# wildminder/ComfyUI-KEEP

Hardware: AMD Instinct MI355X
Metric: restored 512x512 face frames/sec, T=20 clip (higher is better)
Workload: dtype f16x3; 1 GPU; 48 independent clips x T=20 x 512x512 per GPU (BASELINE configs[1] clips), KEEP config, synthetic weights seed 0, precision policy x3; clips_per_gpu=48, clip_length=20, parallelism=dp1 over clips, precision_policy=x3

## Files before the change

comfyui-keep_amd/csrc/keep_conv_x3.hip:

```cpp
#include <stdlib.h>

#include "keep_conv_common.h"

typedef _Float16 f16x8 __attribute__((ext_vector_type(8)));
typedef _Float16 f16x4 __attribute__((ext_vector_type(4)));
typedef unsigned int u32x4 __attribute__((ext_vector_type(4)));
typedef float f32x2 __attribute__((ext_vector_type(2)));
typedef _Float16 f16x2 __attribute__((ext_vector_type(2)));

__device__ __forceinline__ void split4(const float (&v)[4], f16x4& hi, f16x4& lo) {
#pragma unroll
  for (int j = 0; j < 4; ++j) {
    const _Float16 h = (_Float16)v[j];
    hi[j] = h;
    lo[j] = (_Float16)(v[j] - (float)h);
  }
}

template <int PRO, bool FAST>
__device__ __forceinline__ float pro_x3(float v) {
  return FAST ? pro_apply_x3(v, PRO) : pro_apply(v, PRO);
}

typedef unsigned int u32x2 __attribute__((ext_vector_type(2)));
// ... 661 lines not shown
    if (a_mv[it] && (!ONE || p.in_amax || !PLAIN)) {
      a_n[it] = (int)(m / hw);
      const int r = (int)(m - (long)a_n[it] * hw);
      a_oy[it] = r / p.Wo;
      a_ox[it] = r - a_oy[it] * p.Wo;
      if (p.in_amax) {
        float inv;
        x3_range_scale(p.in_amax[a_n[it]], a_s[it], inv);
      }
    }
  }
  const long wrow_stride = (long)p.KH * p.KW * p.Cin * (X1 ? 1 : 2);
  const int b_col = X1 ? (b_pc & 3) * 8 : ((b_pc & 3) >> 1) * XBK + (b_pc >> 2) * 16 + (b_pc & 1) * 8;

  struct StepRegs {
    float a_raw[A_IT][8];
    bool a_ok[A_IT];
    uint4 b_raw[B_IT];
    int a_c;
    float u_sc[8], u_sh[8];
  };
  const long m_last = (m0 + BM - 1 < p.M) ? (m0 + BM - 1) : (long)p.M - 1;
  const bool uni_n = !PLAIN && p.pro_scale && ((m0 / hw) == (m_last / hw));
  const long uni_off = (m0 / hw) * (long)p.Cin;

  const long rows_here = (p.M - m0) < BM ? (p.M - m0) : BM;
  __amdgpu_buffer_rsrc_t a_rsrc = __builtin_amdgcn_make_buffer_rsrc((void*)p.in, 0, 0, 0x00020000);
  int a_voff[A_IT];
  if (ONE) {
    const unsigned long long b = (unsigned long long)(p.in + m0 * p.in_ld);
    const unsigned lo = __builtin_amdgcn_readfirstlane((unsigned)b), hi = __builtin_amdgcn_readfirstlane((unsigned)(b >> 32));
    a_rsrc = __builtin_amdgcn_make_buffer_rsrc((void*)(((unsigned long long)hi << 32) | lo), 0, (int)rows_here * p.in_ld * 4, 0x00020000);
#pragma unroll
    for (int it = 0; it < A_IT; ++it) a_voff[it] = ((a_row0 + it * 64) * p.in_ld + a_grp * 8) * 4;
  }
  __amdgpu_buffer_rsrc_t a2_rsrc = a_rsrc;
  int a2_voff[A_IT];
  const int ld2 = p.Cin - p.cin1;
  if (ONE && p.in2) {
    const unsigned long long b = (unsigned long long)(p.in2 + m0 * ld2);
    const unsigned lo = __builtin_amdgcn_readfirstlane((unsigned)b), hi = __builtin_amdgcn_readfirstlane((unsigned)(b >> 32));
    a2_rsrc = __builtin_amdgcn_make_buffer_rsrc((void*)(((unsigned long long)hi << 32) | lo), 0, (int)rows_here * ld2 * 4, 0x00020000);
#pragma unroll
    for (int it = 0; it < A_IT; ++it) a2_voff[it] = ((a_row0 + it * 64) * ld2 + a_grp * 8) * 4;
  }
  const __amdgpu_buffer_rsrc_t w_rsrc =
      __builtin_amdgcn_make_buffer_rsrc((void*)p.wx3, 0, p.Cout * p.KH * p.KW * p.Cin * (X1 ? 2 : 4), 0x00020000);
  int b_voff[B_IT];
#pragma unroll
  for (int it = 0; it < B_IT; ++it) {
    const int co = n0 + b_row0 + it * 32;
    b_voff[it] = (co < p.Cout && !(X1 && b_pc >= 4)) ? (int)((long)co * wrow_stride * 2) + b_pc * 16 : (int)0x80000000;
  }

  auto fetch = [&](int s, StepRegs& R) {
    const int tap = s / cchunks;
    const int c0 = (s - tap * cchunks) * XBK;
    const int kh = tap / p.KW;
    const int kw = tap - kh * p.KW;
    const int ca = c0 + a_grp * 8;
    R.a_c = ca;
    if (uni_n && ca < p.Cin) {
#pragma unroll
      for (int j = 0; j < 8; ++j) {
        R.u_sc[j] = p.pro_scale[uni_off + ca + j];
        R.u_sh[j] = p.pro_shift[uni_off + ca + j];
      }
    }
    if (ONE) {
#pragma unroll
      for (int it = 0; it < A_IT; ++it) {
        R.a_ok[it] = ca < p.Cin;
        const bool second = p.in2 && c0 >= p.cin1;
        u32x4 v0, v1;
        if (KEEP_LD_AUX_GEMM_A1 != 0 && BN >= 128 && p.Cout <= BN && !p.in2) {
          v0 = __builtin_amdgcn_raw_buffer_load_b128(a_rsrc, a_voff[it], c0 * 4, KEEP_LD_AUX_GEMM_A1);
          v1 = __builtin_amdgcn_raw_buffer_load_b128(a_rsrc, a_voff[it] + 16, c0 * 4, KEEP_LD_AUX_GEMM_A1);
        } else {
          v0 = second ? __builtin_amdgcn_raw_buffer_load_b128(a2_rsrc, a2_voff[it], (c0 - p.cin1) * 4, 0)
                      : __builtin_amdgcn_raw_buffer_load_b128(a_rsrc, a_voff[it], c0 * 4, 0);
          v1 = second ? __builtin_amdgcn_raw_buffer_load_b128(a2_rsrc, a2_voff[it] + 16, (c0 - p.cin1) * 4, 0)
                      : __builtin_amdgcn_raw_buffer_load_b128(a_rsrc, a_voff[it] + 16, c0 * 4, 0);
        }
        R.a_raw[it][0] = __uint_as_float(v0.x); R.a_raw[it][1] = __uint_as_float(v0.y);
        R.a_raw[it][2] = __uint_as_float(v0.z); R.a_raw[it][3] = __uint_as_float(v0.w);
        R.a_raw[it][4] = __uint_as_float(v1.x); R.a_raw[it][5] = __uint_as_float(v1.y);
        R.a_raw[it][6] = __uint_as_float(v1.z); R.a_raw[it][7] = __uint_as_float(v1.w);
      }
    } else {
#pragma unroll
      for (int it = 0; it < A_IT; ++it) {
        int iy = a_oy[it] * p.stride - p.pad_t + kh;
        int ix = a_ox[it] * p.stride - p.pad_l + kw;
        KEEP_REFLECT(iy, ix, p.H, p.W)
        R.a_ok[it] = a_mv[it] && iy >= 0 && iy < p.H && ix >= 0 && ix < p.W && ca < p.Cin;
        if (R.a_ok[it]) {
          const float* src = p.in + (((long)a_n[it] * p.H + iy) * p.W + ix) * p.in_ld + ca;
          const float4 v0 = *reinterpret_cast<const float4*>(src);
          const float4 v1 = *reinterpret_cast<const float4*>(src + 4);
          R.a_raw[it][0] = v0.x; R.a_raw[it][1] = v0.y; R.a_raw[it][2] = v0.z; R.a_raw[it][3] = v0.w;
          R.a_raw[it][4] = v1.x; R.a_raw[it][5] = v1.y; R.a_raw[it][6] = v1.z; R.a_raw[it][7] = v1.w;
        }
      }
    }
    const bool cb_ok = X1 ? c0 + (b_pc & 3) * 8 < p.Cin : c0 + (b_pc >> 2) * 16 < p.Cin;
#pragma unroll
    for (int it = 0; it < B_IT; ++it) {
      const u32x4 v = __builtin_amdgcn_raw_buffer_load_b128(w_rsrc, cb_ok ? b_voff[it] : (int)0x80000000, (tap * p.Cin + c0) * (X1 ? 2 : 4), 0);
      R.b_raw[it] = make_uint4(v.x, v.y, v.z, v.w);
    }
  };

  auto stage = [&](int buf, StepRegs& R) {
#pragma unroll
    for (int it = 0; it < A_IT; ++it) {
      f16x8 hi, lo;
      if (R.a_ok[it]) {
        float v[8];
#pragma unroll
        for (int j = 0; j < 8; ++j) v[j] = R.a_raw[it][j];
        if (!PLAIN) {
          if (uni_n) {
#pragma unroll
            for (int j = 0; j < 8; ++j) v[j] = v[j] * R.u_sc[j] + R.u_sh[j];
          } else if (p.pro_scale) {
            const float* sc = p.pro_scale + (long)a_n[it] * p.Cin + R.a_c;
            const float* sh = p.pro_shift + (long)a_n[it] * p.Cin + R.a_c;
#pragma unroll
            for (int j = 0; j < 8; ++j) v[j] = v[j] * sc[j] + sh[j];
          }
          if (p.pro_act != KEEP_PRO_NONE) {
#pragma unroll
            for (int j = 0; j < 8; ++j) v[j] = p.fast ? pro_apply_x3(v[j], p.pro_act) : pro_apply(v[j], p.pro_act);
          }
        }
#pragma unroll
        for (int j = 0; j < 8; j += 2) {
          const f32x2 vs = f32x2{v[j], v[j + 1]} * a_s[it];
          const f16x2 h = __builtin_convertvector(vs, f16x2);
          hi[j] = h.x; hi[j + 1] = h.y;
          if constexpr (!X1) {
            const f16x2 l = __builtin_convertvector(vs - __builtin_convertvector(h, f32x2), f16x2);
            lo[j] = l.x; lo[j + 1] = l.y;
          }
        }
      } else {
#pragma unroll
        for (int j = 0; j < 8; ++j) { hi[j] = (_Float16)0.f; lo[j] = (_Float16)0.f; }
      }
      _Float16* dst = &As[buf][(a_row0 + it * 64) * XP + a_grp * 8];
      *reinterpret_cast<f16x8*>(dst) = hi;
      if constexpr (!X1) *reinterpret_cast<f16x8*>(dst + XBK) = lo;
    }
    if (X1 && b_pc >= 4) return;
#pragma unroll
    for (int it = 0; it < B_IT; ++it)
      *reinterpret_cast<uint4*>(&Bs[buf][(b_row0 + it * 32) * XP + b_col]) = R.b_raw[it];
  };

  f32x16 acc[TM][TN];
#pragma unroll
  for (int i = 0; i < TM; ++i)
#pragma unroll
    for (int j = 0; j < TN; ++j)
#pragma unroll
      for (int r = 0; r < 16; ++r) acc[i][j][r] = 0.f;

  const int l31 = lane & 31;
  const int lhi = lane >> 5;
  const int a_f0 = (wm * TM * 32 + l31) * XP + lhi * 8;
  const int b_f0 = (wn * TN * 32 + l31) * XP + lhi * 8;

  auto mma_step = [&](int buf, bool zc = false) {
    const _Float16* Ab = As[buf];
    const _Float16* Bb = Bs[buf];
#pragma unroll
    for (int ks = 0; ks < XBK / 16; ++ks) {
      f16x8 ah[TM], al[TM], bh[TN], bl[TN];
#pragma unroll
      for (int i = 0; i < TM; ++i) {
        ah[i] = *reinterpret_cast<const f16x8*>(Ab + a_f0 + i * 32 * XP + ks * 16);
        if constexpr (!X1) al[i] = *reinterpret_cast<const f16x8*>(Ab + a_f0 + i * 32 * XP + ks * 16 + XBK);
      }
#pragma unroll
      for (int j = 0; j < TN; ++j) {
        bh[j] = *reinterpret_cast<const f16x8*>(Bb + b_f0 + j * 32 * XP + ks * 16);
        if constexpr (!X1) bl[j] = *reinterpret_cast<const f16x8*>(Bb + b_f0 + j * 32 * XP + ks * 16 + XBK);
      }
#pragma unroll
      for (int i = 0; i < TM; ++i)
#pragma unroll
        for (int j = 0; j < TN; ++j) {
          if constexpr (X1) {
            acc[i][j] = __builtin_amdgcn_mfma_f32_32x32x16_f16(ah[i], bh[j], acc[i][j], 0, 0, 0);
          } else if (KAL && zc && ks == 0) {
            const f32x16 z16 = {0.f, 0.f, 0.f, 0.f, 0.f, 0.f, 0.f, 0.f, 0.f, 0.f, 0.f, 0.f, 0.f, 0.f, 0.f, 0.f};
            acc[i][j] = __builtin_amdgcn_mfma_f32_32x32x16_f16(al[i], bh[j], z16, 0, 0, 0);
            acc[i][j] = __builtin_amdgcn_mfma_f32_32x32x16_f16(ah[i], bl[j], acc[i][j], 0, 0, 0);
            acc[i][j] = __builtin_amdgcn_mfma_f32_32x32x16_f16(ah[i], bh[j], acc[i][j], 0, 0, 0);
          } else {
            MMA_X3(acc[i][j], ah[i], al[i], bh[j], bl[j])
          }
        }
    }
  };

  if (s_begin < s_end) {
    constexpr int PD = (TM * TN == 1 && DEEP) ? (PLAIN ? 4 : 2) : 1;
    StepRegs R[PD];
#pragma unroll
    for (int u = 0; u < PD; ++u)
      if (s_begin + u < s_end) fetch(s_begin + u, R[u]);
    stage(0, R[0]);
    __syncthreads();
    int buf = 0;
    f32x16 tot[KSL ? TM : 1][KSL ? TN : 1];
    int ksl_left = p.kslice_steps;
    bool ksl_first = true;
    for (int s0 = s_begin; s0 < s_end; s0 += PD) {
#pragma unroll
      for (int u = 0; u < PD; ++u) {
        const int s = s0 + u;
        if (s < s_end) {
          if (s + PD < s_end) fetch(s + PD, R[u]);
          if (KAL) {
            mma_step(buf, u == 0);
            if (u == PD - 1) {
              if (ksl_first) {
#pragma unroll
                for (int i = 0; i < TM; ++i)
#pragma unroll
                  for (int j = 0; j < TN; ++j) tot[KSL ? i : 0][KSL ? j : 0] = acc[i][j];
              } else {
#pragma unroll
                for (int i = 0; i < TM; ++i)
#pragma unroll
                  for (int j = 0; j < TN; ++j)
#pragma unroll
                    for (int r = 0; r < 16; ++r) tot[KSL ? i : 0][KSL ? j : 0][r] += acc[i][j][r];
              }
              ksl_first = false;
            }
          } else {
            mma_step(buf);
          }
          if (KSL && !KAL && --ksl_left == 0) {
            ksl_left = p.kslice_steps;
#pragma unroll
            for (int i = 0; i < TM; ++i)
#pragma unroll
              for (int j = 0; j < TN; ++j)
#pragma unroll
                for (int r = 0; r < 16; ++r) {
                  tot[KSL ? i : 0][KSL ? j : 0][r] = ksl_first ? acc[i][j][r] : tot[KSL ? i : 0][KSL ? j : 0][r] + acc[i][j][r];
                  acc[i][j][r] = 0.f;
                }
            ksl_first = false;
          }
          if (s + 1 < s_end) stage(buf ^ 1, R[(u + 1) % PD]);
          __syncthreads();
          buf ^= 1;
        }
      }
    }
    if (KSL) {
#pragma unroll
      for (int i = 0; i < TM; ++i)
#pragma unroll
        for (int j = 0; j < TN; ++j) acc[i][j] = tot[KSL ? i : 0][KSL ? j : 0];
    }
  }
  const float asc = p.acc_scale;
  if (p.in_amax) {
#pragma unroll
    for (int i = 0; i < TM; ++i)
#pragma unroll
      for (int r = 0; r < 16; ++r) {
        const long m = m0 + wm * TM * 32 + i * 32 + (r & 3) + 8 * (r >> 2) + 4 * lhi;
        float sr = 1.f, inv = 1.f;
        if (m < p.M) x3_range_scale(p.in_amax[m / hw], sr, inv);
#pragma unroll
        for (int j = 0; j < TN; ++j) acc[i][j][r] *= asc * inv;
      }
  } else {
#pragma unroll
    for (int i = 0; i < TM; ++i)
#pragma unroll
      for (int j = 0; j < TN; ++j)
#pragma unroll
        for (int r = 0; r < 16; ++r) acc[i][j][r] *= asc;
  }
  if (m0 + BM <= p.M && p.Cout * 4L * BM < (1L << 30) && p.out_ld * 4L * BM < (1L << 30) && p.res_ld * 4L * BM < (1L << 30)) {
    if (p.split_k == 1 && !p.aux && p.epi_act == KEEP_ACT_NONE)
      x3_gather_epilogue<WGM, WGN, TM, TN, true>(p, acc, reinterpret_cast<float*>(smem_b), m0, n0, wm, wn, lane, wave, z);
    else
      x3_gather_epilogue<WGM, WGN, TM, TN, false>(p, acc, reinterpret_cast<float*>(smem_b), m0, n0, wm, wn, lane, wave, z);
    return;
  }
  staged_epilogue<WGM, WGN, TM, TN>(p, acc, reinterpret_cast<float*>(smem_b), m0, n0, wm, wn, lane, wave, z);
}

#define C3X_K 32
#define C3X_P 72
__global__ __launch_bounds__(256, 2) void conv3x3_c3_x3_kernel(ConvP p, int tiles_x, int tiles_y, int ncb, int n_items) {
  constexpr int HW_ = 34, HROWS = 10;
  constexpr int EPI_B = 4 * 64 * 68 * 4;
  constexpr int A_B = 256 * C3X_P * 2;
  static_assert(A_B + HROWS * HW_ * 4 * 4 <= EPI_B, "im2col rows + halo fit the staging area");
  __shared__ __attribute__((aligned(16))) unsigned char lds_raw[EPI_B + 64 * C3X_P * 2];
  float* et_base = reinterpret_cast<float*>(lds_raw);
  _Float16* As = reinterpret_cast<_Float16*>(lds_raw);
  float* Hs = reinterpret_cast<float*>(lds_raw + A_B);
  _Float16* Ws = reinterpret_cast<_Float16*>(lds_raw + EPI_B);

  const int tid = threadIdx.x;
  const int lane = tid & 63;
  const int wave = tid >> 6;
  const int l31 = lane & 31, lhi = lane >> 5;
  const int Cin = p.Cin, K = 9 * Cin;
  const int rowf = HW_ * Cin;

  int cur_cb = -1;
  auto load_weights = [&](int cb) {
    for (int i = tid; i < 64 * C3X_K; i += 256) {
      const int co = i >> 5, k = i & 31;
      float v = 0.f;
      if (k < K && cb * 64 + co < p.Cout) v = p.w[(long)(cb * 64 + co) * K + k];
      const _Float16 h = (_Float16)v;
      Ws[co * C3X_P + k] = h;
      Ws[co * C3X_P + 32 + k] = (_Float16)(v - (float)h);
    }
  };

  f32x16 acc[2][2];
  const bool has_act = p.epi_act != KEEP_ACT_NONE;
  const int py = tid >> 5, px = tid & 31;
  struct Item { int cb, tx, ty, n; };
  auto decode = [&](int item) {
    Item it;
    const int lid = xcd_remap(item, n_items);
    it.cb = lid % ncb;
    int t = lid / ncb;
    it.tx = t % tiles_x; t /= tiles_x;
    it.ty = t % tiles_y;
    it.n = t / tiles_y;
    return it;
  };
  constexpr int HV = (HROWS * HW_ * 3 + 255) / 256;
  float hv[HV], amax_raw = 0.f;
  auto load_halo = [&](const Item& it) {
    const float* img = p.in + (long)it.n * p.H * p.W * p.in_ld;
    const int oy0 = it.ty * 8, ox0 = it.tx * 32;
#pragma unroll
    for (int u = 0; u < HV; ++u) {
      const int i = tid + u * 256;
      hv[u] = 0.f;
      if (i < HROWS * rowf) {
        const int hy = i / rowf, r = i - hy * rowf;
        const int hx = r / Cin, c = r - hx * Cin;
        const int iy = oy0 - 1 + hy, ix = ox0 - 1 + hx;
        if (iy >= 0 && iy < p.H && ix >= 0 && ix < p.W) hv[u] = img[((long)iy * p.W + ix) * p.in_ld + c];
      }
    }
    if (p.in_amax) amax_raw = p.in_amax[it.n];
  };
  int amax_n = -1;
  float amax_seen = 0.f;
  int item = blockIdx.x;
  if (item >= n_items) return;
  Item nxt = decode(item);
  load_halo(nxt);
  for (; item < n_items; item += gridDim.x) {
    const Item cur = nxt;
    const int cb = cur.cb, tx = cur.tx, ty = cur.ty, n = cur.n;
    const int oy0 = ty * 8, ox0 = tx * 32, n0 = cb * 64;
    float in_s = 1.f, in_inv = 1.f;
    if (p.in_amax) x3_range_scale(amax_raw, in_s, in_inv);
    __syncthreads();
    if (cb != cur_cb) {
      load_weights(cb);
      cur_cb = cb;
    }
#pragma unroll
    for (int u = 0; u < HV; ++u)
      if (tid + u * 256 < HROWS * rowf) Hs[tid + u * 256] = hv[u] * in_s;
    if (item + (int)gridDim.x < n_items) {
      nxt = decode(item + gridDim.x);
      load_halo(nxt);
    }
    __syncthreads();
    {
      float vals[C3X_K];
#pragma unroll
      for (int k = 0; k < C3X_K; ++k) vals[k] = 0.f;
#pragma unroll
      for (int kh = 0; kh < 3; ++kh)
#pragma unroll
        for (int kwc = 0; kwc < 9; ++kwc)
          if (kwc < 3 * Cin && kh * 3 * Cin + kwc < C3X_K) vals[kh * 3 * Cin + kwc] = Hs[(py + kh) * rowf + px * Cin + kwc];
      f16x8 hi[4], lo[4];
#pragma unroll
      for (int k = 0; k < C3X_K; ++k) {
        const _Float16 h = (_Float16)vals[k];
        hi[k >> 3][k & 7] = h;
        lo[k >> 3][k & 7] = (_Float16)(vals[k] - (float)h);
      }
      __syncthreads();
#pragma unroll
      for (int q = 0; q < 4; ++q) {
        *reinterpret_cast<f16x8*>(&As[tid * C3X_P + q * 8]) = hi[q];
        *reinterpret_cast<f16x8*>(&As[tid * C3X_P + 32 + q * 8]) = lo[q];
      }
    }
    __syncthreads();
#pragma unroll
    for (int i = 0; i < 2; ++i)
#pragma unroll
      for (int j = 0; j < 2; ++j)
#pragma unroll
        for (int r = 0; r < 16; ++r) acc[i][j][r] = 0.f;
#pragma unroll
    for (int ks = 0; ks < 2; ++ks) {
      f16x8 ah[2], al[2], bh[2], bl[2];
#pragma unroll
      for (int i = 0; i < 2; ++i) {
        const _Float16* src = &As[(wave * 64 + i * 32 + l31) * C3X_P + ks * 16 + lhi * 8];
        ah[i] = *reinterpret_cast<const f16x8*>(src);
        al[i] = *reinterpret_cast<const f16x8*>(src + 32);
      }
#pragma unroll
      for (int j = 0; j < 2; ++j) {
        const _Float16* src = &Ws[(j * 32 + l31) * C3X_P + ks * 16 + lhi * 8];
        bh[j] = *reinterpret_cast<const f16x8*>(src);
        bl[j] = *reinterpret_cast<const f16x8*>(src + 32);
      }
#pragma unroll
      for (int i = 0; i < 2; ++i)
#pragma unroll
        for (int j = 0; j < 2; ++j) {
          MMA_X3(acc[i][j], ah[i], al[i], bh[j], bl[j])
        }
    }
    __syncthreads();
    constexpr int EP = 68;
    float* et = et_base + wave * 64 * EP;
#pragma unroll
    for (int i = 0; i < 2; ++i)
#pragma unroll
      for (int j = 0; j < 2; ++j)
#pragma unroll
        for (int r = 0; r < 16; ++r) et[(i * 32 + (r & 3) + 8 * (r >> 2) + 4 * lhi) * EP + j * 32 + l31] = acc[i][j][r] * in_inv;
    __builtin_amdgcn_s_waitcnt(0xc07f);
    const int c4 = (lane & 15) * 4, prow = lane >> 4;
    const int co = n0 + c4;
    const bool cok = co < p.Cout;
    float s4[4] = {0.f, 0.f, 0.f, 0.f}, ss4[4] = {0.f, 0.f, 0.f, 0.f};
    float amx = 0.f;
    float4 bias4 = make_float4(0.f, 0.f, 0.f, 0.f);
    if (p.bias && cok) bias4 = *reinterpret_cast<const float4*>(p.bias + co);
#pragma unroll 8
    for (int q16 = 0; q16 < 16; ++q16) {
      if (!cok) break;
      const int pxl = q16 * 4 + prow;
      const int oy = oy0 + 2 * wave + (pxl >> 5);
      const long m = ((long)n * p.Ho + oy) * p.Wo + ox0 + (pxl & 31);
      const float4 v = *reinterpret_cast<const float4*>(et + pxl * EP + c4);
      float e[4] = {v.x + bias4.x, v.y + bias4.y, v.z + bias4.z, v.w + bias4.w};
      if (has_act) {
#pragma unroll
        for (int q = 0; q < 4; ++q) e[q] = p.fast ? act_apply_fast(e[q], p.epi_act) : act_apply(e[q], p.epi_act);
      }
      if (KEEP_NT_C3)
        __builtin_nontemporal_store((f32x4){e[0], e[1], e[2], e[3]}, reinterpret_cast<f32x4*>(p.out + m * p.out_ld + co));
      else
        *reinterpret_cast<float4*>(p.out + m * p.out_ld + co) = make_float4(e[0], e[1], e[2], e[3]);
#pragma unroll
      for (int q = 0; q < 4; ++q) {
        s4[q] += e[q];
        ss4[q] += e[q] * e[q];
        amx = fmaxf(amx, fabsf(e[q]));
      }
    }
    if (p.out_amax) {
      if (n != amax_n) {
        amax_n = n;
        amax_seen = 0.f;
      }
      if (__builtin_amdgcn_ballot_w64(amx > amax_seen) != 0ull) {
        unsigned b = __float_as_uint(amx);
#pragma unroll
        for (int o = 32; o > 0; o >>= 1) b = max(b, (unsigned)__shfl_xor((int)b, o));
        unsigned* dst = p.out_amax + n;
        unsigned seen = b;
        if (lane == 0) {
          seen = *reinterpret_cast<volatile unsigned*>(dst);
          if (b > seen) atomicMax(dst, b);
        }
        seen = max(b, (unsigned)__builtin_amdgcn_readfirstlane((int)seen));
        amax_seen = fmaxf(amax_seen, __uint_as_float(seen));
      }
    }
    if (p.stats) {
#pragma unroll
      for (int q = 0; q < 4; ++q) {
        s4[q] = xor32_sum(xor16_sum(s4[q]));
        ss4[q] = xor32_sum(xor16_sum(ss4[q]));
      }
      if (lane < 16 && cok) {
        float* dst = p.stats + (((long)n * p.stats_P + (ty * tiles_x + tx) * 4 + wave) * p.Cout + co) * 2;
#pragma unroll
        for (int q = 0; q < 4; ++q) {
          dst[q * 2 + 0] = s4[q];
          dst[q * 2 + 1] = ss4[q];
        }
      }
    }
  }
}

int keep_conv2d_x3_c3(const keep_conv2d_args* a, ConvP& p, hipStream_t st, ConvTrace* tr) {
  const int tx = a->Wo / 32, ty = a->Ho / 8, ncb = (a->Cout + 63) / 64;
  const int n_items = a->N * tx * ty * ncb;
  KEEP_CONV_LAUNCH(tr, dim3(persistent_grid(n_items, conv_num_cu(tr))), dim3(256), st, (p, tx, ty, ncb, n_items), conv3x3_c3_x3_kernel);
  KEEP_CONV_LAUNCH_CHECK(tr, "keep_conv2d(Cin<=3, x3)");
  return KEEP_OK;
}

bool keep_conv_x3_halo_ok(const keep_conv2d_args* a) {
  return a->dtype == KEEP_F32 && a->out_dtype != KEEP_BF16 && a->KH == 3 && a->KW == 3 && a->stride == 1 && a->pad_t == 1 &&
         a->pad_l == 1 && (a->Cin % 16 == 0) && (a->Cout % 32 == 0) &&
         ((a->Ho % 8 == 0 && a->Wo % 32 == 0) || (a->Ho % 16 == 0 && a->Wo % 16 == 0)) &&
         a->Ho == (a->upsample ? 2 * a->H : a->H) && a->Wo == (a->upsample ? 2 * a->W : a->W) &&
         (long)a->H * a->W * a->in_ld * 4 < (1L << 31) && (long)a->Cout * 9 * a->Cin * 4 < (1L << 31) &&
         (long)a->Ho * a->Wo * a->out_ld * 4 < (1L << 31) && (long)a->Ho * a->Wo * (a->residual ? a->res_ld : 1) * 4 < (1L << 31) &&
         (!a->pro_scale || ((uintptr_t)a->pro_scale % 16 == 0 && (uintptr_t)a->pro_shift % 16 == 0)) &&
         (a->in_ld % 4 == 0) && ((uintptr_t)a->in % 16 == 0) && (a->out_ld % 4 == 0) && ((uintptr_t)a->out % 16 == 0) &&
         (!a->residual || (a->res_ld % 4 == 0 && (uintptr_t)a->residual % 16 == 0)) &&
         (!a->aux || (uintptr_t)a->aux % 16 == 0) && (!a->bias || (uintptr_t)a->bias % 16 == 0) &&
         (!a->workspace || (uintptr_t)a->workspace % 16 == 0);
}

bool keep_conv_x3_up2_ok(const keep_conv2d_args* a) {
  return keep_conv_x3_halo_ok(a) && a->H % 8 == 0 && a->W % 32 == 0 && a->Cout % 64 == 0 && !a->pro_scale && a->pro_act == KEEP_PRO_NONE &&
         a->epi_act == KEEP_ACT_NONE && !a->aux && a->split_k <= 1 && a->pad_mode == KEEP_PAD_ZERO &&
         (long)4 * a->Cout * 9 * a->Cin * 4 < (1L << 31);
}

bool keep_conv_x3_gather_ok(const keep_conv2d_args* a, const ConvP& p) {
  return a->dtype == KEEP_F32 && a->out_dtype != KEEP_BF16 && !a->upsample && (a->Cin % 16 == 0) && (a->in_ld % 4 == 0) &&
         ((uintptr_t)a->in % 16 == 0) && p.vec_epi && (long)a->Cout * a->KH * a->KW * a->Cin * 4 < (1L << 31);
}

bool keep_conv_x3_gather_is_gemm(const keep_conv2d_args* a) {
  return a->KH == 1 && a->KW == 1 && a->stride == 1 && a->pad_t == 0 && a->pad_l == 0 && a->Ho == a->H && a->Wo == a->W &&
         (long)a->in_ld * 4 * 128 < (1L << 30);
}

bool keep_conv_x1_gather_ok(const keep_conv2d_args* a, const ConvP& p) {
  return keep_conv_x3_gather_ok(a, p) && !keep_conv_x3_gather_is_gemm(a) && !a->pro_scale && a->pro_act == KEEP_PRO_NONE && !a->in2 &&
         !a->ln_gamma && a->Cin % 32 == 0;
}

bool keep_conv_x1_halo16_ok(const keep_conv2d_args* a) {
  return a->dtype == KEEP_F32 && a->out_dtype != KEEP_BF16 && a->KH == 3 && a->KW == 3 && a->stride == 1 && a->pad_t == 1 && a->pad_l == 1 &&
         a->pad_mode == KEEP_PAD_ZERO && !a->upsample && a->Ho == a->H && a->Wo == a->W && a->Ho % 16 == 0 && a->Wo % 16 == 0 &&
         !(a->Ho % 8 == 0 && a->Wo % 32 == 0) && a->Cin % 32 == 0 && a->Cout % 4 == 0 && !a->pro_scale && a->pro_act == KEEP_PRO_NONE &&
         !a->aux && !a->in2 && !a->ln_gamma &&
         (long)a->H * a->W * a->in_ld * 4 < (1L << 31) && (long)a->Cout * 9 * a->Cin * 2 < (1L << 31) &&
         (long)a->Ho * a->Wo * a->out_ld * 4 < (1L << 31) && (long)a->Ho * a->Wo * (a->residual ? a->res_ld : 1) * 4 < (1L << 31) &&
         (a->in_ld % 4 == 0) && ((uintptr_t)a->in % 16 == 0) && (a->out_ld % 4 == 0) && ((uintptr_t)a->out % 16 == 0) &&
         (!a->residual || (a->res_ld % 4 == 0 && (uintptr_t)a->residual % 16 == 0)) && (!a->bias || (uintptr_t)a->bias % 16 == 0);
}

bool keep_conv_x1_gemm_ok(const keep_conv2d_args* a, const ConvP& p) {
  return keep_conv_x3_gather_ok(a, p) && keep_conv_x3_gather_is_gemm(a) && !a->pro_scale && a->pro_act == KEEP_PRO_NONE && !a->in2 &&
         !a->ln_gamma && !a->aux && a->Cin % 32 == 0;
}

enum HaloRun { RUN_SMALL_PARTIALS, RUN_SMALL_FULL, RUN_STREAM, RUN_HALO };

static HaloRun x3_halo_run(const keep_conv2d_args* a, const ConvP& p, const ConvPlan& pl) {
  if (keep_conv_x3p_ok(a, p, p.split_k)) return RUN_SMALL_PARTIALS;
  if (pl.stream) return keep_conv_x3q_ok(a, p, p.split_k) ? RUN_SMALL_FULL : RUN_STREAM;
  if (keep_conv_x3p_full_ok(a, p, p.split_k)) return RUN_SMALL_PARTIALS;
  return RUN_HALO;
}

int keep_conv2d_x3_halo(const keep_conv2d_args* a, ConvP& p, const ConvPlan& pl, hipStream_t st, ConvTrace* tr) {
  const int n_cu = conv_num_cu(tr);
  dim3 block(256);
  if (pl.form == FORM_X1_STREAM) return keep_conv2d_x3_stream(a, p, pl, st, tr);
  if (pl.form == FORM_HALO_UP2) {
    if (pl.stream) return keep_conv2d_x3_up2_stream(a, p, false, st, tr);
    const int tx = a->W / 32, ty = a->H / 8, ncbv = 4 * (a->Cout / 64);
    const int n_items = a->N * tx * ty * ncbv;
    p.upsample = 0;
    dim3 grid(persistent_grid(n_items, n_cu));
    KEEP_CONV_LAUNCH(tr, grid, block, st, (p, tx, ty, ncbv, n_items), conv3x3_halo_x3_kernel<32, KEEP_PRO_NONE, true, true, true, true>);
    KEEP_CONV_LAUNCH_CHECK(tr, "keep_conv2d(halo x3, x2 phases)");
    return KEEP_OK;
  }
  if (pl.form == FORM_X1_UP2) return keep_conv2d_x3_up2_stream(a, p, true, st, tr);
  if (pl.form == FORM_X1_HALO16) {
    const int tiles_x = a->Wo / 16, tiles_y = a->Ho / 16, ncb = (a->Cout + 63) / 64;
    const int n_items = a->N * tiles_x * tiles_y * ncb;
    dim3 grid(persistent_grid(n_items, n_cu));
    if (pl.simple_epi)
      KEEP_CONV_LAUNCH(tr, grid, block, st, (p, tiles_x, tiles_y, ncb, n_items), conv3x3_halo_x3_kernel<16, KEEP_PRO_NONE, true, true, true, false, true>);
    else
      KEEP_CONV_LAUNCH(tr, grid, block, st, (p, tiles_x, tiles_y, ncb, n_items), conv3x3_halo_x3_kernel<16, KEEP_PRO_NONE, false, true, true, false, true>);
    KEEP_CONV_LAUNCH_CHECK(tr, "keep_conv2d(halo x1, 16 x 16 tiles)");
    return KEEP_OK;
  }
  switch (x3_halo_run(a, p, pl)) {
    case RUN_SMALL_PARTIALS: return keep_conv2d_x3_partials(a, p, st, tr);
    case RUN_SMALL_FULL: return keep_conv2d_x3_small_full(a, p, st, tr);
    case RUN_STREAM: return keep_conv2d_x3_stream(a, p, pl, st, tr);
    case RUN_HALO: break;
  }
  const bool wide = pl.wide;
  const int tw = wide ? 32 : 16, th = 256 / tw;
  const int tiles_x = a->Wo / tw, tiles_y = a->Ho / th, ncb = (a->Cout + 63) / 64;
  const int n_items = a->N * tiles_x * tiles_y * ncb * p.split_k;
  dim3 grid(persistent_grid(n_items, n_cu));
  const bool simple = p.split_k == 1 && !a->aux && a->epi_act == KEEP_ACT_NONE;
#define KEEP_LAUNCH_HX2(TWV, PROV)                                                                                          \
  if (simple)                                                                                                              \
    KEEP_CONV_LAUNCH(tr, grid, block, st, (p, tiles_x, tiles_y, ncb, n_items), conv3x3_halo_x3_kernel<TWV, PROV, true, true, true>);  \
  else                                                                                                                     \
    KEEP_CONV_LAUNCH(tr, grid, block, st, (p, tiles_x, tiles_y, ncb, n_items), conv3x3_halo_x3_kernel<TWV, PROV, false, true, true>);
#define KEEP_LAUNCH_HX(TWV)                                       \
  if (a->pro_act == KEEP_PRO_SWISH && !p.fast) {                  \
    if (simple)                                                   \
      KEEP_CONV_LAUNCH(tr, grid, block, st, (p, tiles_x, tiles_y, ncb, n_items), conv3x3_halo_x3_kernel<TWV, KEEP_PRO_SWISH, true, false>);  \
    else                                                          \
      KEEP_CONV_LAUNCH(tr, grid, block, st, (p, tiles_x, tiles_y, ncb, n_items), conv3x3_halo_x3_kernel<TWV, KEEP_PRO_SWISH, false, false>); \
  } else if (a->pro_act == KEEP_PRO_SWISH) {                      \
    KEEP_LAUNCH_HX2(TWV, KEEP_PRO_SWISH)                          \
  } else if (a->pro_act == KEEP_PRO_RELU) {                       \
    KEEP_LAUNCH_HX2(TWV, KEEP_PRO_RELU)                           \
  } else {                                                        \
    KEEP_LAUNCH_HX2(TWV, KEEP_PRO_NONE)                           \
  }
  if (wide) {
    KEEP_LAUNCH_HX(32)
  } else {
    KEEP_LAUNCH_HX(16)
  }
#undef KEEP_LAUNCH_HX
#undef KEEP_LAUNCH_HX2
  KEEP_CONV_LAUNCH_CHECK(tr, "keep_conv2d(halo x3)");
  return KEEP_OK;
}

__global__ __launch_bounds__(256) void conv_x3_gather_stats_replica_kernel(ConvP p) {
  __shared__ float red[4 * 64 * 2];
  const int lane = threadIdx.x & 63, wave = threadIdx.x >> 6;
  const int wm = wave >> 1, wn = wave & 1;
  const long m0 = (long)blockIdx.x * 128;
  const int n0 = blockIdx.y * 128;
  const int c4 = (lane & 15) * 4, prow = lane >> 4;
  const int co = n0 + wn * 64 + c4;
  const bool cok = co < p.Cout;
  float s4[4] = {0.f, 0.f, 0.f, 0.f}, ss4[4] = {0.f, 0.f, 0.f, 0.f};
#pragma unroll 4
  for (int it = 0; it < 16; ++it) {
    const long row = m0 + wm * 64 + it * 4 + prow;
    float4 v = make_float4(0.f, 0.f, 0.f, 0.f);
    if (cok) v = *reinterpret_cast<const float4*>(p.out + row * p.out_ld + co);
    const float e[4] = {v.x, v.y, v.z, v.w};
#pragma unroll
    for (int q = 0; q < 4; ++q) {
      s4[q] += e[q];
      ss4[q] += e[q] * e[q];
    }
  }
#pragma unroll
  for (int q = 0; q < 4; ++q) {
    s4[q] = xor32_sum(xor16_sum(s4[q]));
    ss4[q] = xor32_sum(xor16_sum(ss4[q]));
  }
  if (lane < 16) {
#pragma unroll
    for (int q = 0; q < 4; ++q) {
      red[(wave * 64 + c4 + q) * 2 + 0] = s4[q];
      red[(wave * 64 + c4 + q) * 2 + 1] = ss4[q];
    }
  }
  __syncthreads();
  const int hw_o = p.Ho * p.Wo;
  const int n_img = (int)(m0 / hw_o), p_idx = (int)((m0 % hw_o) / 128);
  for (int c = threadIdx.x; c < 128; c += 256) {
    const int wn_c = c >> 6, rem = c & 63;
    float a = 0.f, b2 = 0.f;
#pragma unroll
    for (int mm = 0; mm < 2; ++mm) {
      a += red[((mm * 2 + wn_c) * 64 + rem) * 2 + 0];
      b2 += red[((mm * 2 + wn_c) * 64 + rem) * 2 + 1];
    }
    if (n0 + c < p.Cout) {
      float* dst = p.stats + (((long)n_img * p.stats_P + p_idx) * p.Cout + n0 + c) * 2;
      dst[0] = a;
      dst[1] = b2;
    }
  }
}

static constexpr long KEEP_GATHER_SMALL_ROWS = 4096;
int keep_conv2d_x3_gather(const keep_conv2d_args* a, ConvP& p, const ConvPlan& pl, hipStream_t st, ConvTrace* tr) {
  const long M = p.M;
  const bool ln = pl.form == FORM_GEMM_LN, x1 = pl.form == FORM_X1_IM2COL || pl.form == FORM_X1_GEMM;
  bool big_tile = pl.tile == 2;
  float* replica_stats = nullptr;
  if (big_tile && p.stats && M <= KEEP_GATHER_SMALL_ROWS && M % 128 == 0 && ((long)p.Ho * p.Wo) % 128 == 0 && p.split_k == 1 && p.vec_epi &&
      p.Cout % 4 == 0 && !p.out_bf16 && !(a->flags & KEEP_CONV_NO_SMALL_PARTIALS)) {
    replica_stats = p.stats;
    p.stats = nullptr;
    big_tile = false;
  }
  if (big_tile && !ln && !p.stats && M <= KEEP_GATHER_SMALL_ROWS) big_tile = false;
  const int steps = a->KH * a->KW * ((a->Cin + XBK - 1) / XBK);
  const bool plain = pl.plain;
  dim3 block(256);
  const bool one = pl.gemm;
#define KEEP_LAUNCH_GX(A, B, C, D)                                                                 \
  if (x1 && one)                                                                                   \
    KEEP_CONV_LAUNCH(tr, grid, block, st, (p), conv_x3_kernel<A, B, C, D, true, true, false, true, false, true>); \
  else if (x1)                                                                                     \
    KEEP_CONV_LAUNCH(tr, grid, block, st, (p), conv_x3_kernel<A, B, C, D, true, false, false, true, false, true>); \
  else if (p.kslice_steps == 4 && plain && C * D == 1 && steps % 4 == 0)                                \
    KEEP_CONV_LAUNCH(tr, grid, block, st, (p), conv_x3_kernel<A, B, C, D, true, true, true, true, C * D == 1>); \
  else if (p.kslice_steps > 0 && plain)                                                            \
    KEEP_CONV_LAUNCH(tr, grid, block, st, (p), conv_x3_kernel<A, B, C, D, true, true, true>);     \
  else if (p.kslice_steps > 0)                                                                     \
    KEEP_CONV_LAUNCH(tr, grid, block, st, (p), conv_x3_kernel<A, B, C, D, false, true, true>);    \
  else if (plain && one)                                                                           \
    KEEP_CONV_LAUNCH(tr, grid, block, st, (p), conv_x3_kernel<A, B, C, D, true, true>);           \
  else if (plain && C * D == 1 && M > 262144)                                                      \
    KEEP_CONV_LAUNCH(tr, grid, block, st, (p), conv_x3_kernel<A, B, C, D, true, false, false, false>); \
  else if (plain)                                                                                  \
    KEEP_CONV_LAUNCH(tr, grid, block, st, (p), conv_x3_kernel<A, B, C, D, true, false>);          \
  else if (one)                                                                                    \
    KEEP_CONV_LAUNCH(tr, grid, block, st, (p), conv_x3_kernel<A, B, C, D, false, true>);          \
  else                                                                                             \
    KEEP_CONV_LAUNCH(tr, grid, block, st, (p), conv_x3_kernel<A, B, C, D, false, false>);
  const int bt = big_tile ? 128 : 64;
  const long gx = cdiv(M, bt), gy = cdiv(a->Cout, bt);
  const bool rowmajor = gy > 1 && gx >= 1024 && gx * gy < (1L << 30);
  p.tile_cols = rowmajor ? (int)gy : 0;
  dim3 grid(rowmajor ? (unsigned)(gx * gy) : (unsigned)gx, rowmajor ? 1u : (unsigned)gy, p.split_k);
  if (ln) {
    KEEP_CONV_LAUNCH(tr, grid, block, st, (p), conv_x3_kernel<4, 1, 1, 4, true, true>);
  } else if (!big_tile) {
    KEEP_LAUNCH_GX(2, 2, 1, 1)
  } else {
    KEEP_LAUNCH_GX(2, 2, 2, 2)
  }
#undef KEEP_LAUNCH_GX
  KEEP_CONV_LAUNCH_CHECK(tr, "keep_conv2d(gather x3)");
  if (replica_stats) {
    p.stats = replica_stats;
    KEEP_CONV_LAUNCH(tr, dim3((unsigned)(M / 128), (unsigned)cdiv(a->Cout, 128)), dim3(256), st, (p), conv_x3_gather_stats_replica_kernel);
    KEEP_CONV_LAUNCH_CHECK(tr, "keep_conv2d(gather x3, statistics replica)");
  }
  return KEEP_OK;
}
```

Measured before the change: 301.6 frames/s.

## Gather im2col from halo directly into registers and double-buffer the halo

Reworks the Cin<=3 x3 first-layer conv kernel. It drops the shared-memory im2col staging: each wave now gathers its A fragments straight from the halo using a precomputed offset table, splits them into hi/lo f16 in registers, and processes one output row at a time, so the per-wave epilogue tile halves. The halo is double-buffered, so only one block barrier per item is needed, plus another only when the weights change. Halo index math is hoisted out of the loop. Smaller LDS use lets launch bounds rise to 3 blocks per CU with a matching resident grid size, at the cost of more register pressure and scattered LDS reads.

New measurement: 302.1 frames/s (median of 6 runs). No clear change (+0.2%).

```diff
diff --git a/comfyui-keep_amd/csrc/keep_conv_x3.hip b/comfyui-keep_amd/csrc/keep_conv_x3.hip
--- a/comfyui-keep_amd/csrc/keep_conv_x3.hip
+++ b/comfyui-keep_amd/csrc/keep_conv_x3.hip
@@ -987,16 +987,15 @@
 
 #define C3X_K 32
 #define C3X_P 72
-__global__ __launch_bounds__(256, 2) void conv3x3_c3_x3_kernel(ConvP p, int tiles_x, int tiles_y, int ncb, int n_items) {
-  constexpr int HW_ = 34, HROWS = 10;
-  constexpr int EPI_B = 4 * 64 * 68 * 4;
-  constexpr int A_B = 256 * C3X_P * 2;
-  static_assert(A_B + HROWS * HW_ * 4 * 4 <= EPI_B, "im2col rows + halo fit the staging area");
-  __shared__ __attribute__((aligned(16))) unsigned char lds_raw[EPI_B + 64 * C3X_P * 2];
-  float* et_base = reinterpret_cast<float*>(lds_raw);
-  _Float16* As = reinterpret_cast<_Float16*>(lds_raw);
-  float* Hs = reinterpret_cast<float*>(lds_raw + A_B);
-  _Float16* Ws = reinterpret_cast<_Float16*>(lds_raw + EPI_B);
+#define C3X_HB 1024
+#define C3X_BLOCKS_PER_CU 3
+__global__ __launch_bounds__(256, C3X_BLOCKS_PER_CU) void conv3x3_c3_x3_kernel(ConvP p, int tiles_x, int tiles_y, int ncb, int n_items) {
+  constexpr int HW_ = 34, HROWS = 10, EP = 68;
+  static_assert(HROWS * HW_ * 3 <= C3X_HB, "the halo fits its buffer");
+  __shared__ __attribute__((aligned(16))) float et_all[4 * 32 * EP];
+  __shared__ __attribute__((aligned(16))) float Hs2[2 * C3X_HB];
+  __shared__ __attribute__((aligned(16))) _Float16 Ws[64 * C3X_P];
+  __shared__ __attribute__((aligned(16))) int Ao[C3X_K];
 
   const int tid = threadIdx.x;
   const int lane = tid & 63;
@@ -1017,9 +1016,12 @@
     }
   };
 
-  f32x16 acc[2][2];
   const bool has_act = p.epi_act != KEEP_ACT_NONE;
-  const int py = tid >> 5, px = tid & 31;
+  if (tid < C3X_K) {
+    const int k = ((tid >> 3) & 1) * 16 + (tid >> 4) * 8 + (tid & 7);
+    const int kh = k / (3 * Cin);
+    Ao[tid] = k < K ? kh * rowf + (k - kh * 3 * Cin) : -1;
+  }
   struct Item { int cb, tx, ty, n; };
   auto decode = [&](int item) {
     Item it;
@@ -1033,19 +1035,24 @@
   };
   constexpr int HV = (HROWS * HW_ * 3 + 255) / 256;
   float hv[HV], amax_raw = 0.f;
+  int h_y[HV], h_x[HV], h_off[HV];
+#pragma unroll
+  for (int u = 0; u < HV; ++u) {
+    const int i = tid + u * 256;
+    const int hy = i / rowf, r = i - hy * rowf;
+    const int hx = r / Cin;
+    h_y[u] = i < HROWS * rowf ? hy : -1;
+    h_x[u] = hx;
+    h_off[u] = hx * p.in_ld + (r - hx * Cin);
+  }
   auto load_halo = [&](const Item& it) {
     const float* img = p.in + (long)it.n * p.H * p.W * p.in_ld;
     const int oy0 = it.ty * 8, ox0 = it.tx * 32;
 #pragma unroll
     for (int u = 0; u < HV; ++u) {
-      const int i = tid + u * 256;
       hv[u] = 0.f;
-      if (i < HROWS * rowf) {
-        const int hy = i / rowf, r = i - hy * rowf;
-        const int hx = r / Cin, c = r - hx * Cin;
-        const int iy = oy0 - 1 + hy, ix = ox0 - 1 + hx;
-        if (iy >= 0 && iy < p.H && ix >= 0 && ix < p.W) hv[u] = img[((long)iy * p.W + ix) * p.in_ld + c];
-      }
+      const int iy = oy0 - 1 + h_y[u], ix = ox0 - 1 + h_x[u];
+      if (h_y[u] >= 0 && iy >= 0 && iy < p.H && ix >= 0 && ix < p.W) hv[u] = img[((long)iy * p.W + (ox0 - 1)) * p.in_ld + h_off[u]];
     }
     if (p.in_amax) amax_raw = p.in_amax[it.n];
   };
@@ -1055,116 +1062,102 @@
   if (item >= n_items) return;
   Item nxt = decode(item);
   load_halo(nxt);
-  for (; item < n_items; item += gridDim.x) {
+  float* const et = et_all + wave * 32 * EP;
+  const int c4 = (lane & 15) * 4, prow = lane >> 4;
+  for (int buf = 0; item < n_items; item += gridDim.x, buf ^= 1) {
     const Item cur = nxt;
     const int cb = cur.cb, tx = cur.tx, ty = cur.ty, n = cur.n;
     const int oy0 = ty * 8, ox0 = tx * 32, n0 = cb * 64;
     float in_s = 1.f, in_inv = 1.f;
     if (p.in_amax) x3_range_scale(amax_raw, in_s, in_inv);
-    __syncthreads();
-    if (cb != cur_cb) {
+    const bool new_w = cb != cur_cb;
+    if (new_w) {
+      __syncthreads();
       load_weights(cb);
       cur_cb = cb;
     }
+    float* Hs = Hs2 + buf * C3X_HB;
 #pragma unroll
     for (int u = 0; u < HV; ++u)
-      if (tid + u * 256 < HROWS * rowf) Hs[tid + u * 256] = hv[u] * in_s;
+      if (h_y[u] >= 0) Hs[tid + u * 256] = hv[u] * in_s;
     if (item + (int)gridDim.x < n_items) {
       nxt = decode(item + gridDim.x);
       load_halo(nxt);
     }
     __syncthreads();
-    {
-      float vals[C3X_K];
-#pragma unroll
-      for (int k = 0; k < C3X_K; ++k) vals[k] = 0.f;
-#pragma unroll
-      for (int kh = 0; kh < 3; ++kh)
-#pragma unroll
-        for (int kwc = 0; kwc < 9; ++kwc)
-          if (kwc < 3 * Cin && kh * 3 * Cin + kwc < C3X_K) vals[kh * 3 * Cin + kwc] = Hs[(py + kh) * rowf + px * Cin + kwc];
-      f16x8 hi[4], lo[4];
-#pragma unroll
-      for (int k = 0; k < C3X_K; ++k) {
-        const _Float16 h = (_Float16)vals[k];
-        hi[k >> 3][k & 7] = h;
-        lo[k >> 3][k & 7] = (_Float16)(vals[k] - (float)h);
-      }
-      __syncthreads();
-#pragma unroll
-      for (int q = 0; q < 4; ++q) {
-        *reinterpret_cast<f16x8*>(&As[tid * C3X_P + q * 8]) = hi[q];
-        *reinterpret_cast<f16x8*>(&As[tid * C3X_P + 32 + q * 8]) = lo[q];
-      }
-    }
-    __syncthreads();
-#pragma unroll
-    for (int i = 0; i < 2; ++i)
-#pragma unroll
-      for (int j = 0; j < 2; ++j)
-#pragma unroll
-        for (int r = 0; r < 16; ++r) acc[i][j][r] = 0.f;
-#pragma unroll
-    for (int ks = 0; ks < 2; ++ks) {
-      f16x8 ah[2], al[2], bh[2], bl[2];
-#pragma unroll
-      for (int i = 0; i < 2; ++i) {
-        const _Float16* src = &As[(wave * 64 + i * 32 + l31) * C3X_P + ks * 16 + lhi * 8];
-        ah[i] = *reinterpret_cast<const f16x8*>(src);
-        al[i] = *reinterpret_cast<const f16x8*>(src + 32);
-      }
-#pragma unroll
-      for (int j = 0; j < 2; ++j) {
-        const _Float16* src = &Ws[(j * 32 + l31) * C3X_P + ks * 16 + lhi * 8];
-        bh[j] = *reinterpret_cast<const f16x8*>(src);
-        bl[j] = *reinterpret_cast<const f16x8*>(src + 32);
-      }
-#pragma unroll
-      for (int i = 0; i < 2; ++i)
-#pragma unroll
-        for (int j = 0; j < 2; ++j) {
-          MMA_X3(acc[i][j], ah[i], al[i], bh[j], bl[j])
-        }
-    }
-    __syncthreads();
-    constexpr int EP = 68;
-    float* et = et_base + wave * 64 * EP;
-#pragma unroll
-    for (int i = 0; i < 2; ++i)
-#pragma unroll
-      for (int j = 0; j < 2; ++j)
-#pragma unroll
-        for (int r = 0; r < 16; ++r) et[(i * 32 + (r & 3) + 8 * (r >> 2) + 4 * lhi) * EP + j * 32 + l31] = acc[i][j][r] * in_inv;
-    __builtin_amdgcn_s_waitcnt(0xc07f);
-    const int c4 = (lane & 15) * 4, prow = lane >> 4;
     const int co = n0 + c4;
     const bool cok = co < p.Cout;
     float s4[4] = {0.f, 0.f, 0.f, 0.f}, ss4[4] = {0.f, 0.f, 0.f, 0.f};
     float amx = 0.f;
     float4 bias4 = make_float4(0.f, 0.f, 0.f, 0.f);
     if (p.bias && cok) bias4 = *reinterpret_cast<const float4*>(p.bias + co);
-#pragma unroll 8
-    for (int q16 = 0; q16 < 16; ++q16) {
-      if (!cok) break;
-      const int pxl = q16 * 4 + prow;
-      const int oy = oy0 + 2 * wave + (pxl >> 5);
-      const long m = ((long)n * p.Ho + oy) * p.Wo + ox0 + (pxl & 31);
-      const float4 v = *reinterpret_cast<const float4*>(et + pxl * EP + c4);
-      float e[4] = {v.x + bias4.x, v.y + bias4.y, v.z + bias4.z, v.w + bias4.w};
-      if (has_act) {
-#pragma unroll
-        for (int q = 0; q < 4; ++q) e[q] = p.fast ? act_apply_fast(e[q], p.epi_act) : act_apply(e[q], p.epi_act);
-      }
-      if (KEEP_NT_C3)
-        __builtin_nontemporal_store((f32x4){e[0], e[1], e[2], e[3]}, reinterpret_cast<f32x4*>(p.out + m * p.out_ld + co));
-      else
-        *reinterpret_cast<float4*>(p.out + m * p.out_ld + co) = make_float4(e[0], e[1], e[2], e[3]);
-#pragma unroll
-      for (int q = 0; q < 4; ++q) {
-        s4[q] += e[q];
-        ss4[q] += e[q] * e[q];
-        amx = fmaxf(amx, fabsf(e[q]));
-      }
+#pragma unroll
+    for (int i = 0; i < 2; ++i) {
+      int lh = lhi;
+      asm volatile("" : "+v"(lh));
+      const float* hp = Hs + (2 * wave + i) * rowf + l31 * Cin;
+      f16x8 ah[2], al[2], bh[2][2], bl[2][2];
+#pragma unroll
+      for (int ks = 0; ks < 2; ++ks) {
+        const int4 o0 = *reinterpret_cast<const int4*>(&Ao[lh * 16 + ks * 8]), o1 = *reinterpret_cast<const int4*>(&Ao[lh * 16 + ks * 8 + 4]);
+        const int o[8] = {o0.x, o0.y, o0.z, o0.w, o1.x, o1.y, o1.z, o1.w};
+#pragma unroll
+        for (int e = 0; e < 8; ++e) {
+          const float raw = hp[max(o[e], 0)];
+          const float v = o[e] >= 0 ? raw : 0.f;
+          const _Float16 h = (_Float16)v;
+          ah[ks][e] = h;
+          al[ks][e] = (_Float16)(v - (float)h);
+        }
+#pragma unroll
+        for (int j = 0; j < 2; ++j) {
+          const _Float16* src = &Ws[(j * 32 + l31) * C3X_P + ks * 16 + lh * 8];
+          bh[ks][j] = *reinterpret_cast<const f16x8*>(src);
+          bl[ks][j] = *reinterpret_cast<const f16x8*>(src + 32);
+        }
+      }
+      f32x16 acc[2];
+#pragma unroll
+      for (int j = 0; j < 2; ++j)
+#pragma unroll
+        for (int r = 0; r < 16; ++r) acc[j][r] = 0.f;
+#pragma unroll
+      for (int ks = 0; ks < 2; ++ks)
+#pragma unroll
+        for (int j = 0; j < 2; ++j) {
+          MMA_X3(acc[j], ah[ks], al[ks], bh[ks][j], bl[ks][j])
+        }
+#pragma unroll
+      for (int j = 0; j < 2; ++j)
+#pragma unroll
+        for (int r = 0; r < 16; ++r) et[((r & 3) + 8 * (r >> 2) + 4 * lhi) * EP + j * 32 + l31] = acc[j][r] * in_inv;
+      __builtin_amdgcn_s_waitcnt(0xc07f);
+      __builtin_amdgcn_wave_barrier();
+      if (cok) {
+        const long m0 = ((long)n * p.Ho + oy0 + 2 * wave + i) * p.Wo + ox0;
+#pragma unroll
+        for (int q8 = 0; q8 < 8; ++q8) {
+          const int pxl = q8 * 4 + prow;
+          const long m = m0 + pxl;
+          const float4 v = *reinterpret_cast<const float4*>(et + pxl * EP + c4);
+          float e[4] = {v.x + bias4.x, v.y + bias4.y, v.z + bias4.z, v.w + bias4.w};
+          if (has_act) {
+#pragma unroll
+            for (int q = 0; q < 4; ++q) e[q] = p.fast ? act_apply_fast(e[q], p.epi_act) : act_apply(e[q], p.epi_act);
+          }
+          if (KEEP_NT_C3)
+            __builtin_nontemporal_store((f32x4){e[0], e[1], e[2], e[3]}, reinterpret_cast<f32x4*>(p.out + m * p.out_ld + co));
+          else
+            *reinterpret_cast<float4*>(p.out + m * p.out_ld + co) = make_float4(e[0], e[1], e[2], e[3]);
+#pragma unroll
+          for (int q = 0; q < 4; ++q) {
+            s4[q] += e[q];
+            ss4[q] += e[q] * e[q];
+            amx = fmaxf(amx, fabsf(e[q]));
+          }
+        }
+      }
+      __builtin_amdgcn_wave_barrier();
     }
     if (p.out_amax) {
       if (n != amax_n) {
@@ -1206,7 +1199,8 @@
 int keep_conv2d_x3_c3(const keep_conv2d_args* a, ConvP& p, hipStream_t st, ConvTrace* tr) {
   const int tx = a->Wo / 32, ty = a->Ho / 8, ncb = (a->Cout + 63) / 64;
   const int n_items = a->N * tx * ty * ncb;
-  KEEP_CONV_LAUNCH(tr, dim3(persistent_grid(n_items, conv_num_cu(tr))), dim3(256), st, (p, tx, ty, ncb, n_items), conv3x3_c3_x3_kernel);
+  const int resident = C3X_BLOCKS_PER_CU * conv_num_cu(tr);
+  KEEP_CONV_LAUNCH(tr, dim3(n_items < resident ? n_items : resident), dim3(256), st, (p, tx, ty, ncb, n_items), conv3x3_c3_x3_kernel);
   KEEP_CONV_LAUNCH_CHECK(tr, "keep_conv2d(Cin<=3, x3)");
   return KEEP_OK;
 }
```
